# nikhilTkur/Multigrid_dolfinx

Measured on AMD Instinct MI355X. Metric: V-cycles/sec + achieved HBM GB/s, 3D Poisson P1 1024³ DoF, 1/2/4/8 MI355X, higher is better.
Workload: dtype f64

## Files before the change

### multigrid_dolfinx_amd/csrc/mg_capi.hip

```cpp
#include "../../include/mg_hip.h"
#include "mg_kernels.hip.h"
#include "mg_direct.hip.h"
#include "mg_jacobi2.hip.h"
#include "mg_jacobik3d.hip.h"
#include "mg_jacobiblk.hip.h"
#include "mg_lattice.hip.h"

#include <dlfcn.h>
#include <rccl/rccl.h>

#include <algorithm>
#include <array>
#include <cmath>
#include <cstdio>
#include <cstdlib>
#include <cstring>
#include <string>
#include <vector>

using namespace mgk;

namespace {

thread_local std::string g_err;
// ... 174 lines not shown
    int restriction = MG_RESTRICT_INJECTION, smoother = MG_SMOOTH_JACOBI;
    double coarse_rtol = 1e-14;
    int coarse_maxit = 20000;
    int keep_err = 0;
    int use_codes = 1;
    int use_sdia = 1;
    int strip_slices = 64;
    int nontemporal = 1;
    int lds_pad = 32768;
    int rows_per_lane = 2;
    unsigned chunk = 8;
    int pcg_chunk = 16;
    double* partials = nullptr;
    double* scalars = nullptr;
    int* done = nullptr;
    double* h_scalars = nullptr;
    double *pcg_r = nullptr, *pcg_z = nullptr, *pcg_q = nullptr, *pcg_part_a = nullptr, *pcg_part_b = nullptr;
    DVector pcg_p;
    int pcg_parts = 0, pcg_parts_a = 0;
    int pcg_predict = 0;
    int use_graph = 1;
    int comm_priority = 1;
    int lattice_march = 1;
    int64_t lattice_march_min_rows = 1 << 22;
    int lattice_gs2 = 0;
    int lattice_tile = 0;
    int lattice_segments = 0;
    int slab_pair_form = 0;
    int graph_comm = 0;
    uint64_t epoch = 1;
    std::vector<CycleGraph> graphs;
    int use_direct = 1;
    int require_diagonal = 1;
    int fuse_restrict = 1;
    int fuse_block = 1;
    int64_t fuse_block_min_rows = (int64_t)1 << 15, fuse_block_max_rows = (int64_t)1 << 23;
    int fuse_block_k = 0, fuse_block_ez = 11;
    int direct_block_rows = 2048;
    int fuse_2d_lines = 0;
    int gen_odd_rows = 0;
    int cls_escape = 1;
    int storage_auto = 1;
    int storage_qbits = 0;
    int use_classes = 1;
    int fuse_sweeps = 1;
    int64_t fuse_min_rows = (int64_t)1 << 24;
    int fuse_segments = 0;
    int fuse_nontemporal = 0;
    int fuse_classes = 1;
    int fuse_plain_shape = 0;
    int fuse_plain = 2;
    int class_sweeps = 1;
    int fuse_k = 5;
    int fuse_k_shape = 7;
    int fuse_k_segments = 0;
    int timing_force_form = -1;
    int64_t fuse_k_slab_min_rows = (int64_t)1 << 20;
    int fuse_k_slab_min_sweeps = 4;
    int64_t fuse_k_min_rows = (int64_t)1 << 24;
    int64_t fuse_k_small_rows = (int64_t)1 << 22;
    int64_t fuse_k5_min_rows = (int64_t)1 << 26;
    int64_t fuse_k4_min_rows = 0;
    int fuse_k_nt_store = 0;
    int fuse_k_tail = 1;
    int fuse_k_small_tiles = 0;
    int fuse_k_pf = 1;
    int fuse_k_dpp = 1;
    std::vector<const void*> large_lds_kernels;
    int fuse_shape = 1;
    int fuse_wi = 0;
    int fuse_even = 0;
    int march_sweeps = 1;
    int64_t march_min_rows = (int64_t)1 << 22;
    int march_shape = 0;
    int64_t fuse_small_2d_rows = 2048;
    int fuse_small = 1;
    int fuse_2d = 1;
    int fuse_2d_k = 5;
    int fuse_xcd_chunk = 32;
    int cls_blocks_per_cu = 4;
    DirectSolver direct;
    int* ptab_count = nullptr;
    int* rtab_count = nullptr;
    int* rtab_off = nullptr;
    double* rtab_w = nullptr;
    int rtab_m = 0;
    int* ptab_off = nullptr;
    double* ptab_w = nullptr;
    Level mass;
    int mass_level = -1;
    DVector mass_out, diff, uexact;
    int uexact_level = -1;
    int64_t uploads = 0, downloads = 0, graph_replays = 0;
    struct SmootherCount { int64_t launches = 0, sweeps = 0, tail = 0; };
    std::vector<std::array<SmootherCount, MG_PATH_COUNT>> smoother_counts;
    int jk3_tail = 0;
    double* stage = nullptr;
    int64_t stage_elems = 0;
    int64_t bytes = 0;
    Comm comm;
    hipDeviceProp_t prop{};
};

namespace {

constexpr int kMaxParts = 1024;

// ... 876 lines not shown
    L.cls_halo = 1;
    return 0;
}

bool sweepsk_ok(const mg_context* c, const Level& L, bool ignore_size = false) {
    if (c->fuse_k < 3 || !L.cls || !c->fuse_classes) return false;
    if (L.cls_escape) {
        if (L.esc_kmax < 3) return false;
        ignore_size = true;
    }
    const bool slab = !L.replicated && c->comm.active();
    if (slab && (L.hd < 2 || L.cls_halo < 0 || c->halo_planes != 1)) return false;
    if (!ignore_size && (slab ? min_slab_rows(L) < c->fuse_k_slab_min_rows : L.nloc < c->fuse_k_min_rows)) return false;
    return fused_sweeps_ok(c, L, true) && L.g.nk >= 8;
}

int sweepsk_max(const mg_context* c, const Level& L) {
    const int k = std::min(std::min(c->fuse_k, 5), L.nloc < c->fuse_k4_min_rows ? 3 : L.nloc < c->fuse_k_small_rows ? 5 : L.nloc < c->fuse_k5_min_rows ? 4 : 5);
    return L.cls_escape ? std::min(k, L.esc_kmax) : k;
}

template <int K>
int escape_window_k(mg_context* c, const Level& L, const unsigned char* cls, int64_t clead, unsigned* most) {
    constexpr int WI = 64 - 2 * K, HY = 16 * 2 - 2 * K + 2;
    JK3WindowArgs a{};
    a.cls = cls; a.clead = clead; a.P = L.g.plane; a.nx = L.g.nx; a.ny = L.g.ny; a.nz = L.g.nk;
    a.ntx = (a.nx + WI - 1) / WI; a.nty = (a.ny + HY - 1) / HY;
    a.most = reinterpret_cast<unsigned*>(c->partials);
    HIP_TRY(hipMemsetAsync(a.most, 0, sizeof(unsigned), c->stream));
    hipLaunchKernelGGL((jk3_escape_window<K, 16, 2, 1>), dim3((unsigned)(a.ntx * a.nty)), dim3(256), 0, c->stream, a);
    HIP_TRY(hipGetLastError());
    HIP_TRY(hipMemcpyAsync(most, a.most, sizeof(unsigned), hipMemcpyDeviceToHost, c->stream));
    HIP_TRY(hipStreamSynchronize(c->stream));
    if (std::getenv("MG_DEBUG_STORAGE"))
        std::fprintf(stderr, "[mg] escape rows: at most %u in %d planes of a tile (%d sweeps per pass, pool of %d)\n", *most, K + 2, K, jk3_pool(K));
    return 0;
}

int escape_kmax(mg_context* c, const Level& L, const unsigned char* cls, int64_t clead, int* kmax) {
    *kmax = 0;
    if (L.wu != 4 || L.g.nk < 8 || L.g.nx < 32 || L.g.ny < 32) return 0;
    unsigned most = 0;
    MG_TRY(escape_window_k<5>(c, L, cls, clead, &most));
    if (most <= (unsigned)jk3_pool(5)) { *kmax = 5; return 0; }
    MG_TRY(escape_window_k<4>(c, L, cls, clead, &most));
    if (most <= (unsigned)jk3_pool(4)) { *kmax = 4; return 0; }
    MG_TRY(escape_window_k<3>(c, L, cls, clead, &most));
    if (most <= (unsigned)jk3_pool(3)) *kmax = 3;
    return 0;
}

struct JK3Range { int za0, za1, zb0, zb1; };

template <int K, int NW, int LPW, int M, bool DPP, int PF = 1, int WPE = (NW == 12 ? 3 : 2), int TR = 256, bool ESC = false>
int launch_jacobikc_t(mg_context* c, JK3Args a, bool finest, const JK3Range& zr, int seglen) {
    constexpr int EX = 64 * M, EY = NW * LPW, WI = EX - 2 * K, HY = EY - 2 * K + 2;
    a.ntx = (a.nx + WI - 1) / WI;
    a.nty = (a.ny + HY - 1) / HY;
    const int64_t ntile = (int64_t)a.ntx * a.nty;
    constexpr size_t lds = jk3_lds_bytes<K, NW, LPW, M, TR, ESC>();
    static_assert(lds <= 160 * 1024, "one CU's LDS");
    a.za0 = zr.za0; a.za1 = zr.za1; a.zb0 = zr.zb0; a.zb1 = zr.zb1;
    const int planes = std::max(0, zr.za1 - zr.za0) + std::max(0, zr.zb1 - zr.zb0);
    if (planes <= 0) return 0;
    a.ta = (int)ntile; a.seglen_b = 1;
    int64_t items = 0;
    if (seglen <= 0) {
        int64_t cus = std::max(1, c->prop.multiProcessorCount) * (int64_t)std::max<size_t>(1, std::min<size_t>(160 * 1024 / lds, (size_t)(4 * WPE / NW)));
        if (c->fuse_k_tail > 1) cus = c->fuse_k_tail;
        const double warm = 1.4 * K;
        int best = 1, best_ta = (int)ntile, best_m = 1;
        double best_cost = 1e300;
        const bool tail = c->fuse_k_tail && zr.zb1 <= zr.zb0;
        for (int n = 1; n <= std::max(1, planes / 8); ++n) {
            const int len = (planes + n - 1) / n;
            const int64_t full = ntile * n / cus;
            int64_t ta = tail ? std::min<int64_t>(ntile, full * cus / n) : ntile;
            if (ta <= 0 || (ntile - ta) * 2 > cus) ta = ntile;
            const int64_t tb = ntile - ta;
            const int m = tb > 0 ? (int)std::max<int64_t>(1, std::min<int64_t>(cus / tb, planes / 4)) : 1;
            const double cost = (double)((ta * n + cus - 1) / cus) * (len + warm) + (tb > 0 ? (planes + m - 1) / m + warm : 0.0);
            if (cost < best_cost) { best_cost = cost; best = n; best_ta = (int)ta; best_m = m; }
        }
        if (c->fuse_k_segments > 0) { best = std::min(c->fuse_k_segments, planes); best_ta = (int)ntile; }
        seglen = (planes + best - 1) / best;
        a.ta = best_ta;
        a.seglen_b = best_ta < ntile ? (planes + best_m - 1) / best_m : 1;
    }
    a.seglen = seglen;
    {
        const int nseg = (std::max(0, zr.za1 - zr.za0) + seglen - 1) / seglen + (std::max(0, zr.zb1 - zr.zb0) + seglen - 1) / seglen;
        items = (int64_t)a.ta * nseg;
        if (a.ta < ntile) items += (ntile - a.ta) * (int64_t)((planes + a.seglen_b - 1) / a.seglen_b);
    }
    if (items >= ((int64_t)1 << 31) - 4096) return fail("too many tiles");
    a.nitems = (unsigned)items;
    a.xcd_chunk = (unsigned)c->fuse_xcd_chunk;
    const int64_t group = 8 * (int64_t)a.xcd_chunk;
    const unsigned grid = (unsigned)(((items + group - 1) / group) * group);
    if (a.ncls > TR) return fail("more row classes than this tile shape keeps in LDS");
    void (*kern)(JK3Args) = finest ? sdia_jacobikc_finest<K, NW, LPW, M, DPP, PF, WPE, TR> : sdia_jacobikc<K, NW, LPW, M, DPP, PF, WPE, TR>;
    if constexpr (ESC) kern = sdia_jacobikc_escape<K, NW, LPW, M, DPP, PF, WPE, TR>;
    MG_TRY(allow_large_lds(c, reinterpret_cast<const void*>(kern), lds));
    hipLaunchKernelGGL(kern, dim3(grid), dim3(NW * WAVE), lds, c->stream, a);
    HIP_TRY(hipGetLastError());
    c->jk3_tail = a.ta < ntile ? 1 : 0;
    return 0;
}

template <int K, int PF>
int launch_jacobikc_kp(mg_context* c, const JK3Args& a, bool finest, const JK3Range& zr, int seglen) {
    if (!c->fuse_k_dpp) return launch_jacobikc_t<K, 12, 2, 2, false, PF>(c, a, finest, zr, seglen);
    int shape = c->fuse_k_shape >= 3 && a.ncls > 64 ? 1 : c->fuse_k_shape;
    if (shape == 1 && a.ncls <= 64 && K <= 4 && c->fuse_k_small_tiles) {
        constexpr int WI = 64 - 2 * K, HY = 48 - 2 * K + 2;
        if ((int64_t)((a.nx + WI - 1) / WI) * ((a.ny + HY - 1) / HY) < std::max(1, c->prop.multiProcessorCount)) shape = 4;
    }
    switch (shape) {
        case 1: return launch_jacobikc_t<K, 12, 4, 1, true, PF>(c, a, finest, zr, seglen);
        case 2: return launch_jacobikc_t<K, 8, 3, 2, true, PF>(c, a, finest, zr, seglen);
        case 3: return launch_jacobikc_t<K, 6, 4, 1, true, PF, 3, 64>(c, a, finest, zr, seglen);
        case 4: return launch_jacobikc_t<K, 8, 3, 1, true, PF, 4, 64>(c, a, finest, zr, seglen);
        case 5: if constexpr (K <= 4) return launch_jacobikc_t<K, 4, 6, 1, true, PF, 2, 64>(c, a, finest, zr, seglen);
        case 6: if constexpr (K <= 4 && PF == 1) return launch_jacobikc_t<K, 16, 3, 1, true, 1, 4>(c, a, finest, zr, seglen);
        case 7: return launch_jacobikc_t<K, 16, 2, 1, true, PF, 4>(c, a, finest, zr, seglen);
        default: return launch_jacobikc_t<K, 12, 2, 2, true, PF>(c, a, finest, zr, seglen);
    }
}

template <int K>
int launch_jacobikc_k(mg_context* c, const JK3Args& a, bool finest, const JK3Range& zr, int seglen) {
    if (a.escape) {
        if constexpr (K >= 3) return launch_jacobikc_t<K, 16, 2, 1, true, 1, 4, 256, true>(c, a, finest, zr, seglen);
        else return fail("levels with escape rows take three to five sweeps per pass");
    }
    if constexpr (K == 3 || K == 4) {
        if (c->fuse_k_pf == 2 && (K == 3 || c->fuse_k_shape == 7)) return launch_jacobikc_kp<K, 2>(c, a, finest, zr, seglen);
    }
    if constexpr (K == 2) return launch_jacobikc_t<K, 12, 4, 1, true, 1>(c, a, finest, zr, seglen);
    else return launch_jacobikc_kp<K, 1>(c, a, finest, zr, seglen);
}

int launch_jacobikc(mg_context* c, const Level& L, int K, const double* x_rows, const double* f_rows, double* out_rows,
                    const JK3Range* zr = nullptr, int seglen = 0) {
    JK3Args a{};
    a.x = x_rows; a.f = f_rows; a.out = out_rows;
    a.cls = L.cls; a.ctab = L.ctab; a.clead = L.cls_lead; a.ncls = L.ncls; a.cmain = L.cmain;
    for (int t = 0; t < 8; ++t) a.cm[t] = L.cm[t];
    a.P = L.g.plane; a.nx = L.g.nx; a.ny = L.g.ny; a.nz = L.g.nk; a.omega = c->omega;
    const bool dist = !L.replicated && c->comm.active();
    a.plo = dist && c->comm.rank > 0 ? K : 0;
    a.phi = dist && c->comm.rank + 1 < c->comm.world ? K : 0;
    if (dist && (L.hd < K || L.cls_halo != 1)) return fail("the level's halos are not prepared for that many sweeps per pass");
    if (L.cls_escape && K > L.esc_kmax) return fail("too many escape rows per tile for that many sweeps per pass");
    a.force_form = c->timing_force_form;
    a.nt_store = c->fuse_k_nt_store;
    a.escape = L.cls_escape ? 1 : 0; a.dvals = L.dvals; a.mlead = L.mlead; a.sshift = L.R == 1 ? 6 : (L.R == 2 ? 7 : 8);
    const JK3Range whole{0, L.g.nk, 0, 0};
    const bool finest = c->nlev > 1 && &L == &c->L[c->nlev - 1];
    c->jk3_tail = 0;
    switch (K) {
        case 2: return launch_jacobikc_k<2>(c, a, finest, zr ? *zr : whole, seglen);
        case 3: return launch_jacobikc_k<3>(c, a, finest, zr ? *zr : whole, seglen);
        case 4: return launch_jacobikc_k<4>(c, a, finest, zr ? *zr : whole, seglen);
        case 5: return launch_jacobikc_k<5>(c, a, finest, zr ? *zr : whole, seglen);
        default: return fail("sweeps per pass must be in 2..5");
    }
}

int check_coloring(mg_context* c, Level& L) {
    EllArgs a{};
    a.vals = L.vals; a.cols = L.cols; a.codes = L.codes; a.offsets = L.offsets; a.W = L.W;
    a.nloc = L.nloc; a.lead = L.g.lead; a.dinv = L.dinv; a.color_kind = COLOR_LATTICE9; a.grow0 = L.row0; a.gnx = L.g.nx; a.gny = L.g.ny;
    int* d_flag = reinterpret_cast<int*>(c->partials);
    HIP_TRY(hipMemsetAsync(d_flag, 0, sizeof(int), c->stream));
    const dim3 grid(blocks_for(L.nloc, 256)), blk(256);
    if (L.sdia) {
        a.vals = L.dvals; a.mlead = L.mlead;
        for (int t = 0; t < 8; ++t) a.up[t] = L.up[t];
        switch (L.R) {
            case 1: hipLaunchKernelGGL(sdia_check_coloring<1>, grid, blk, 0, c->stream, a, L.wu, d_flag); break;
            case 2: hipLaunchKernelGGL(sdia_check_coloring<2>, grid, blk, 0, c->stream, a, L.wu, d_flag); break;
            default: hipLaunchKernelGGL(sdia_check_coloring<4>, grid, blk, 0, c->stream, a, L.wu, d_flag); break;
        }
    } else {
        switch (L.R) {
            case 1: hipLaunchKernelGGL(ell_check_coloring<1>, grid, blk, 0, c->stream, a, L.nslices, d_flag); break;
            case 2: hipLaunchKernelGGL(ell_check_coloring<2>, grid, blk, 0, c->stream, a, L.nslices, d_flag); break;
            default: hipLaunchKernelGGL(ell_check_coloring<4>, grid, blk, 0, c->stream, a, L.nslices, d_flag); break;
        }
// ... 1600 lines not shown
    } else if (k == "fuse_shape") {
        if (value < 0 || value > 3) return fail("fuse_shape must be 0..3");
        c->fuse_shape = (int)value;
    } else if (k == "march_sweeps") {
        c->march_sweeps = value != 0;
    } else if (k == "march_min_rows") {
        c->march_min_rows = value;
    } else if (k == "march_shape") {
        if (value < 0 || value > 1) return fail("march_shape must be 0 or 1");
        c->march_shape = (int)value;
    } else if (k == "fuse_small_2d_rows") {
        c->fuse_small_2d_rows = value;
    } else if (k == "fuse_small") {
        c->fuse_small = value != 0;
    } else if (k == "fuse_2d") {
        c->fuse_2d = value != 0;
    } else if (k == "fuse_2d_k") {
        if (value < 2 || value > 5) return fail("fuse_2d_k must be in 2..5");
        c->fuse_2d_k = (int)value;
    } else if (k == "lattice_march") {
        c->lattice_march = value != 0;
    } else if (k == "lattice_march_min_rows") {
        c->lattice_march_min_rows = value;
    } else if (k == "lattice_gs2") {
        c->lattice_gs2 = value != 0;
    } else if (k == "lattice_tile") {
        if (value < 0 || value > 2) return fail("lattice_tile must be 0, 1 or 2");
        c->lattice_tile = (int)value;
    } else if (k == "lattice_segments") {
        if (value < 0 || value > 4096) return fail("lattice_segments must be in 0..4096");
        c->lattice_segments = (int)value;
    } else if (k == "fuse_xcd_chunk") {
        if (value < 1 || value > 512) return fail("fuse_xcd_chunk must be in 1..512");
        c->fuse_xcd_chunk = (int)value;
    } else if (k == "cls_blocks_per_cu") {
        if (value < 1 || value > 64) return fail("cls_blocks_per_cu must be in 1..64");
        c->cls_blocks_per_cu = (int)value;
    } else if (k == "fuse_wi") {
        c->fuse_wi = (int)value;
    } else if (k == "fuse_even") {
        c->fuse_even = value != 0;
    } else if (k == "class_sweeps") {
        c->class_sweeps = value != 0;
    } else if (k == "fuse_plain_shape") {
        if (value < 0 || value > 2) return fail("fuse_plain_shape must be 0..2");
        c->fuse_plain_shape = (int)value;
    } else if (k == "fuse_plain") {
        if (value != 1 && value != 2) return fail("fuse_plain must be 1 or 2");
        c->fuse_plain = (int)value;
    } else if (k == "fuse_k") {
        if (value < 0 || value > 5) return fail("fuse_k must be in 0..5 (below 3: pairs of sweeps only)");
        c->fuse_k = (int)value;
    } else if (k == "fuse_k_shape") {
        if (value < 0 || value > 7) return fail("fuse_k_shape must be 0..7");
        c->fuse_k_shape = (int)value;
    } else if (k == "fuse_k_slab_min_rows") {
        c->fuse_k_slab_min_rows = value;
    } else if (k == "fuse_k_slab_min_sweeps") {
        if (value < 2) return fail("fuse_k_slab_min_sweeps must be at least 2");
        c->fuse_k_slab_min_sweeps = (int)value;
    } else if (k == "fuse_k_min_rows") {
        c->fuse_k_min_rows = value;
    } else if (k == "fuse_k_small_rows") {
        c->fuse_k_small_rows = value;
    } else if (k == "fuse_k5_min_rows") {
        c->fuse_k5_min_rows = value;
    } else if (k == "fuse_k4_min_rows") {
        c->fuse_k4_min_rows = value;
    } else if (k == "fuse_k_nt_store") {
        c->fuse_k_nt_store = value != 0;
    } else if (k == "fuse_k_tail") {
        if (value < 0) return fail("fuse_k_tail must be >= 0");
        c->fuse_k_tail = (int)value;
    } else if (k == "fuse_k_small_tiles") {
        c->fuse_k_small_tiles = value != 0;
    } else if (k == "fuse_k_pf") {
        if (value != 1 && value != 2) return fail("fuse_k_pf must be 1 or 2");
        c->fuse_k_pf = (int)value;
    } else if (k == "fuse_k_dpp") {
        c->fuse_k_dpp = value != 0;
    } else if (k == "fuse_k_segments") {
        if (value < 0) return fail("fuse_k_segments must be >= 0");
        c->fuse_k_segments = (int)value;
    } else if (k == "fuse_classes") {
        c->fuse_classes = value != 0;
    } else if (k == "fuse_nontemporal") {
        c->fuse_nontemporal = value != 0;
    } else if (k == "fuse_segments") {
        if (value < 0) return fail("fuse_segments must be >= 0");
        c->fuse_segments = (int)value;
    } else if (k == "coarse_direct") {
        c->use_direct = value != 0;
        free_direct(c);
    } else if (k == "pcg_chunk") {
        if (value < 1) return fail("pcg_chunk must be positive");
        c->pcg_chunk = (int)value;
    } else {
        return fail("unknown tuning key " + k);
    }
    return 0;
}

namespace {

struct DevTemp {
    void* p = nullptr;
    DevTemp() = default;
// ... 823 lines not shown
```

### multigrid_dolfinx_amd/csrc/mg_jacobik3d.hip.h

```cpp
#pragma once
#include "mg_jacobi2.hip.h"
#include <type_traits>

namespace mgk {

struct JK3Args {
    const double* x;
    const double* f;
    double* out;
    const unsigned char* cls;
    const double* ctab;
    int64_t clead, P;
    int ncls, cmain;
    double cm[8];
    double omega;
    int nx, ny, nz;
    int plo, phi;
    int ntx, nty, seglen, za0, za1, zb0, zb1;
    int ta, seglen_b;
    unsigned nitems, xcd_chunk;
    int nt_store;
    int escape;
    const double* dvals;
    int64_t mlead;
    int sshift;
    int force_form;
};

constexpr int jk3_pool(int K) { return K >= 5 ? 512 : 1024; }

template <int K, int NW, int LPW, int M, int TR> constexpr size_t jk3_lds_doubles() {
    return TR * CLS_W + (size_t)K * (NW * LPW + 2) * (64 * M) + 2 * (64 * M + 2);
}
template <int K, int NW, int LPW, int M, int TR, bool ESC = false> constexpr size_t jk3_lds_bytes() {
    constexpr size_t base = jk3_lds_doubles<K, NW, LPW, M, TR>();
    return sizeof(double) * (ESC ? (base + CLS_W - 1) / CLS_W * CLS_W + (size_t)(jk3_pool(K) + 1) * CLS_W : base);
}


template <int K, int NW, int LPW, int M, bool DPP, int PF, int TR, bool ESC = false>
__device__ __forceinline__ void jk3_body(const JK3Args& a) {
    constexpr int EX = 64 * M, EY = NW * LPW, NC = M * LPW, IMG = (EY + 2) * EX;
    constexpr int CBITS = ESC ? 16 : 8, CPR = 32 / CBITS, CW = (NC + CPR - 1) / CPR;
    constexpr unsigned CMASK = (1u << CBITS) - 1u;
    constexpr int DYN0 = (int)((jk3_lds_doubles<K, NW, LPW, M, TR>() + CLS_W - 1) / CLS_W);
    static_assert(CLS_W == 8, "table rows of eight doubles");
    constexpr int WI = EX - 2 * K, HY = EY - 2 * K + 2;
    static_assert(NC * (K + 1) <= 64, "the fast-path flags live in one scalar register pair");
    static_assert(WI > 0 && HY > 0, "tile too small for K sweeps");
    static_assert(PF == 1 || PF == 2, "planes of x in flight");
    extern __shared__ double j2_smem[];
    double* const sT = j2_smem;
    double* const sI = sT + TR * CLS_W + (EX + 2);
    const int lane = threadIdx.x & 63;
    const int wave = __builtin_amdgcn_readfirstlane((int)(threadIdx.x >> 6));

    unsigned id;
    {
        const unsigned b = blockIdx.x, xcd = b & 7u, j = b >> 3, ch = a.xcd_chunk;
        id = ((j / ch) * 8u + xcd) * ch + (j % ch);
    }
    if (id >= a.nitems) return;
    const unsigned ntile = (unsigned)(a.ntx * a.nty);
    const int nsa = (a.za1 - a.za0 + a.seglen - 1) / a.seglen;
    const int nsb = (a.zb1 - a.zb0 + a.seglen - 1) / a.seglen;
    const unsigned items_a = (unsigned)a.ta * (unsigned)(nsa + max(nsb, 0));
    unsigned tt;
    int z0, z1;
    if (id < items_a) {
        const int seg = (int)(id / (unsigned)a.ta);
        tt = id % (unsigned)a.ta;
        z0 = seg < nsa ? a.za0 + seg * a.seglen : a.zb0 + (seg - nsa) * a.seglen;
        z1 = min(seg < nsa ? a.za1 : a.zb1, z0 + a.seglen);
    } else {
        const unsigned j = id - items_a, tb = ntile - (unsigned)a.ta;
        tt = (unsigned)a.ta + j % tb;
        z0 = a.za0 + (int)(j / tb) * a.seglen_b;
        z1 = min(a.za1, z0 + a.seglen_b);
    }
    const int tiy = (int)(tt / (unsigned)a.ntx), tix = (int)(tt % (unsigned)a.ntx);
    if (z1 <= z0) return;
    const int tx0 = tix * WI - K, ty0 = tiy * HY - (K - 1);

    {
        const int nt = a.ncls * CLS_W;
        for (int i = threadIdx.x; i < nt; i += NW * WAVE) {
            double v = a.ctab[i];
            if ((i & (CLS_W - 1)) == CLS_W - 1) {
                const double d = a.ctab[i - 4];
                v = a.omega * (1.0 / (d != 0.0 ? d : 1.0));
            }
            sT[i] = v;
        }
        for (int i = threadIdx.x; i < K * IMG + 2 * (EX + 2); i += NW * WAVE) sT[TR * CLS_W + i] = 0.0;
    }
    unsigned* const esc_count = reinterpret_cast<unsigned*>(sT + (size_t)CLS_W * (DYN0 + jk3_pool(K)));
    if constexpr (ESC) {
        if (threadIdx.x == 0) *esc_count = 0u;
    }
    const double m0 = a.cm[0], m1 = a.cm[1], m2 = a.cm[2], m3 = a.cm[3], m4 = a.cm[4], m5 = a.cm[5], m6 = a.cm[6];
    const double mcf = a.omega * (1.0 / (m3 != 0.0 ? m3 : 1.0));
    const int cmain = a.cmain;

    const int ey0 = wave * LPW;
    const int lw0 = (ey0 + 1) * EX + lane;
    auto lwof = [&](int c) -> int { return (c / M) * EX + 64 * (c % M); };
    int ibase[(K + 1) / 2];
#pragma unroll
    for (int q = 0; q < (K + 1) / 2; ++q) {
        ibase[q] = 2 * q * IMG + lw0;
        asm volatile("" : "+v"(ibase[q]));
    }
    auto image = [&](int t) -> double* { return sI + ibase[t >> 1] + (t & 1) * IMG; };
    unsigned inT = 0;
    const int64_t rb0 = (int64_t)(ty0 + ey0) * a.nx + (tx0 + lane);
    auto rowof = [&](int c) -> int64_t { return rb0 + (int64_t)(c / M) * a.nx + 64 * (c % M); };
    unsigned shw = 0;
#pragma unroll
    for (int c = 0; c < NC; ++c) {
        const int ex = lane + 64 * (c % M), ey = ey0 + c / M;
        if (ex >= K && ex < EX - K && ey >= K - 1 && ey <= EY - K && tx0 + ex < a.nx && ty0 + ey < a.ny) inT |= 1u << c;
        const int64_t r = rowof(c);
        shw |= (r < 0 ? 0u : (r >= a.P ? 2u : 1u)) << (2 * c);
    }
    auto shof = [&](int c) -> int { return (int)((shw >> (2 * c)) & 3u) - 1; };
    unsigned standin = 0;
#pragma unroll
    for (int c = 0; c < NC; ++c) {
        const int line = ty0 + ey0 + c / M;
        if (lane + 64 * (c % M) > a.nx + 1 - tx0 || line < -2 || line > a.ny + 1) standin |= 1u << c;
    }
    const bool wlo = wave == 0, whi = wave == NW - 1;

    const int bias = 2 * a.nx + K + 2;
    const int xcl = a.nx + 1 - tx0;
    unsigned eo[NC], eor[M];
#pragma unroll
    for (int c = 0; c < NC; ++c)
        eo[c] = 8u * (unsigned)(min(max(ty0 + ey0 + c / M, -2), a.ny + 1) * a.nx + tx0 + min(lane + 64 * (c % M), xcl) + bias);
#pragma unroll
    for (int r = 0; r < M; ++r)
        eor[r] = 8u * (unsigned)((wlo ? max(ty0 - 1, -2) : min(ty0 + EY, a.ny + 1)) * a.nx + tx0 + min(lane + 64 * r, xcl) + bias);
    const unsigned char* const clsb = a.cls + a.clead - bias;
    const double* const xb0 = a.x - bias;
    const double* const fb0 = a.f - bias;
    auto sbase = [](const void* p) -> gcptr_t {
        const unsigned long long u = (unsigned long long)p;
        const unsigned lo = (unsigned)__builtin_amdgcn_readfirstlane((int)(unsigned)u);
        const unsigned hi = (unsigned)__builtin_amdgcn_readfirstlane((int)(unsigned)(u >> 32));
        return (gcptr_t)(((unsigned long long)hi << 32) | lo);
    };
    auto ldd = [](gcptr_t b, unsigned e8) -> double {
        asm volatile("" : "+v"(e8));
        return *(const __attribute__((address_space(1))) double*)(b + e8);
    };
    typedef unsigned int __attribute__((aligned(1))) u32_unaligned_t;
    auto ldc = [](gcptr_t b, unsigned e8) -> int {
        unsigned e = e8 >> 3;
        asm volatile("" : "+v"(e));
        return (int)*(const __attribute__((address_space(1))) u32_unaligned_t*)(b + e);
    };
    const int pmin = -a.plo - 1, pmax = a.nz + a.phi;

    double acc[K][NC], fr[K][NC];
    double XA[NC], XB[PF == 2 ? NC : 1], hyA[M], hyB[PF == 2 ? M : 1];
    int CA[NC], CB[PF == 2 ? NC : 1];
    double FN[PF == 2 ? NC : 1];
    unsigned cw[K + 1][CW];
    unsigned long long fast = 0;
    constexpr unsigned long long ALLFAST = (NC * (K + 1) == 64) ? ~0ull : ((1ull << (NC * (K + 1))) - 1ull);
#pragma unroll
    for (int c = 0; c < NC; ++c) {
#pragma unroll
        for (int t = 0; t < K; ++t) acc[t][c] = fr[t][c] = 0.0;
        XA[c] = 0.0;
        CA[c] = 0;
    }
#pragma unroll
    for (int j = 0; j <= K; ++j)
#pragma unroll
        for (int q = 0; q < CW; ++q) cw[j][q] = 0u;
#pragma unroll
    for (int r = 0; r < M; ++r) hyA[r] = 0.0;
    XB[0] = 0.0; hyB[0] = 0.0; CB[0] = 0; FN[0] = 0.0;

    auto load_slice = [&](const int i, const int n, const int plane, const int fplane, double (&X)[NC], int (&C)[NC], double (&hy)[M])
        __attribute__((always_inline)) {
        const int64_t o = (int64_t)min(max(plane, pmin), pmax) * a.P;
        const gcptr_t cb = sbase(clsb + o);
        const gcptr_t xb = sbase(xb0 + o);
        const gcptr_t fb = sbase(fb0 + (int64_t)min(max(fplane, pmin), pmax) * a.P);
#pragma unroll
        for (int c = 0; c < NC; ++c) {
            if ((c * n) / NC != i) continue;
            X[c] = ldd(xb, eo[c]);
            C[c] = ldc(cb, eo[c]);
            if constexpr (PF == 2) FN[c] = ldd(fb, eo[c]);
            else fr[K - 1][c] = ldd(fb, eo[c]);
        }
        if (i == n - 1 && (wlo || whi)) {
#pragma unroll
            for (int r = 0; r < M; ++r) hy[r] = ldd(xb, eor[r]);
        }
    };
    auto cls_of = [&](int j, int c) -> int { return (int)((cw[j][c / CPR] >> (CBITS * (c % CPR))) & CMASK); };
    auto cls_now = [&](int j, int c) -> int {
        unsigned w = cw[j][c / CPR];
        asm volatile("" : "+v"(w));
        return (int)((w >> (CBITS * (c % CPR))) & CMASK);
    };
    int k_plane = 0;
    bool k_store = false;
    __attribute__((address_space(1))) char* k_out = nullptr;
    auto store = [&](int c, double v) {
        unsigned e8 = eo[c];
        asm volatile("" : "+v"(e8));
        if (a.nt_store) __builtin_nontemporal_store(v, (__attribute__((address_space(1))) double*)(k_out + e8));
        else *(__attribute__((address_space(1))) double*)(k_out + e8) = v;
    };
    int lo_t[K + 1], n_t[K + 1];
#pragma unroll
    for (int t = 1; t <= K; ++t) {
        lo_t[t] = -min(a.plo, K - t);
        n_t[t] = a.nz + min(a.phi, K - t) - lo_t[t];
    }

    auto phase_a_fast = [&](auto col_tag, const double (&X)[NC]) __attribute__((always_inline)) {
        constexpr bool COL = decltype(col_tag)::value;
#pragma unroll
        for (int r = 0; r < M; ++r) {
#pragma unroll
            for (int l = 0; l < LPW; ++l) {
                const int c = l * M + r, iw = lwof(c);
                double k0 = m0, k6 = m6, kcf = mcf;
                if constexpr (COL) {
                    const dvec2_t* const tr = reinterpret_cast<const dvec2_t*>(sT + CLS_W * cls_of(0, c));
                    const dvec2_t t01 = tr[0], t67 = tr[3];
                    k0 = t01.x; k6 = t67.x; kcf = t67.y;
                }
                double nw = X[c];
#pragma unroll
                for (int t = 1; t <= K; ++t) {
                    double* const img = image(t - 1);
                    const double wd = img[iw];
                    const double s = fma(k6, nw, acc[t - 1][c]);
                    const double o = wd + kcf * (fr[K - t][c] - s);
                    acc[t - 1][c] = fma(k0, wd, 0.0);
                    img[iw] = nw;
                    nw = o;
                }
                if (k_store && (inT >> c & 1u)) store(c, nw);
            }
        }
    };
    auto phase_b_fast = [&](auto col_tag, const int t) __attribute__((always_inline)) {
        constexpr bool COL = decltype(col_tag)::value;
        const double* const img = image(t - 1);
        double v[LPW][M], ys[M], yn[M];
#pragma unroll
        for (int r = 0; r < M; ++r) {
            ys[r] = img[-EX + 64 * r];
#pragma unroll
            for (int l = 0; l < LPW; ++l) v[l][r] = img[l * EX + 64 * r];
            yn[r] = img[LPW * EX + 64 * r];
        }
#pragma unroll
        for (int l = 0; l < LPW; ++l) {
            double yw[M], ye[M];
            if constexpr (DPP) {
                double fw[M], fe[M];
#pragma unroll
                for (int r = 0; r < M; ++r) { fw[r] = jk3_from_west(v[l][r]); fe[r] = jk3_from_east(v[l][r]); }
#pragma unroll
                for (int r = 0; r < M; ++r) {
                    yw[r] = (r > 0 && lane == 0) ? fw[r > 0 ? r - 1 : 0] : fw[r];
                    ye[r] = (r + 1 < M && lane == 63) ? fe[r + 1 < M ? r + 1 : r] : fe[r];
                }
            } else {
#pragma unroll
                for (int r = 0; r < M; ++r) {
                    yw[r] = img[l * EX + 64 * r - 1];
                    ye[r] = img[l * EX + 64 * r + 1];
                }
            }
#pragma unroll
            for (int r = 0; r < M; ++r) {
                const int c = l * M + r;
                double k1 = m1, k2 = m2, k3 = m3, k4 = m4, k5 = m5;
                if constexpr (COL) {
                    const dvec2_t* const tr = reinterpret_cast<const dvec2_t*>(sT + CLS_W * cls_of(0, c));
                    const dvec2_t t01 = tr[0], t23 = tr[1], t45 = tr[2];
                    k1 = t01.y; k2 = t23.x; k3 = t23.y; k4 = t45.x; k5 = t45.y;
                }
                double s = acc[t - 1][c];
                s = fma(k1, l > 0 ? v[l > 0 ? l - 1 : 0][r] : ys[r], s);
                s = fma(k2, yw[r], s);
                s = fma(k3, v[l][r], s);
                s = fma(k4, ye[r], s);
                s = fma(k5, l + 1 < LPW ? v[l + 1 < LPW ? l + 1 : l][r] : yn[r], s);
                acc[t - 1][c] = s;
            }
        }
    };
    auto phase_a_general = [&](const double (&X)[NC]) __attribute__((always_inline)) {
#pragma unroll
        for (int c = 0; c < NC; ++c) {
            const int iw = lwof(c);
            double nw = X[c];
            int pc = k_plane + shof(c);
            asm volatile("" : "+v"(pc));
#pragma unroll
            for (int t = 1; t <= K; ++t) {
                const int j = K - t;
                double* const img = image(t - 1);
                const double wd = img[iw];
                const dvec2_t t67 = reinterpret_cast<const dvec2_t*>(sT + CLS_W * cls_now(j, c))[3];
                const dvec2_t t01 = reinterpret_cast<const dvec2_t*>(sT + CLS_W * cls_now(j + 1, c))[0];
                const double s = fma(t67.x, nw, acc[t - 1][c]);
                double o = wd + t67.y * (fr[j][c] - s);
                o = (unsigned)(pc + j - lo_t[t]) < (unsigned)n_t[t] ? o : 0.0;
                acc[t - 1][c] = fma(t01.x, wd, 0.0);
                img[iw] = nw;
                nw = o;
                __builtin_amdgcn_sched_barrier(0);
            }
            if (k_store && (inT >> c & 1u)) store(c, nw);
        }
    };
    auto phase_b_general = [&](const int t) __attribute__((always_inline)) {
#pragma unroll
        for (int c = 0; c < NC; ++c) {
            const int iw = lwof(c);
            const double* const img = image(t - 1);
            const double ys = img[iw - EX], yw = img[iw - 1], yd = img[iw], ye = img[iw + 1], yn = img[iw + EX];
            const dvec2_t* const tr = reinterpret_cast<const dvec2_t*>(sT + CLS_W * cls_now(K - t, c));
            const dvec2_t t01 = tr[0], t23 = tr[1], t45 = tr[2];
            double s = acc[t - 1][c];
            s = fma(t01.y, ys, s);
            s = fma(t23.x, yw, s);
            s = fma(t23.y, yd, s);
            s = fma(t45.x, ye, s);
            s = fma(t45.y, yn, s);
            acc[t - 1][c] = s;
            __builtin_amdgcn_sched_barrier(0);
        }
    };

    auto step = [&](const int k, double (&X)[NC], int (&C)[NC], double (&hy)[M], double (&XN)[PF == 2 ? NC : 1],
                    int (&CN)[PF == 2 ? NC : 1], double (&hyN)[PF == 2 ? M : 1]) __attribute__((always_inline)) {
        k_plane = k; k_store = k >= z0;
        {
            const unsigned long long u = (unsigned long long)(a.out - bias + (int64_t)k * a.P);
            const unsigned lo = (unsigned)__builtin_amdgcn_readfirstlane((int)(unsigned)u);
            const unsigned hi = (unsigned)__builtin_amdgcn_readfirstlane((int)(unsigned)(u >> 32));
            k_out = (__attribute__((address_space(1))) char*)(((unsigned long long)hi << 32) | lo);
        }
#pragma unroll
        for (int c = 0; c < NC; ++c) {
            asm volatile("" : "+v"(C[c]));
            asm volatile("" : "+v"(X[c]));
            C[c] &= 255;
        }
        if constexpr (ESC) {
            if (a.escape) {
                const int64_t mp = (int64_t)min(max(k + K, pmin), pmax) * a.P - bias + a.mlead;
                const int sh = a.sshift;
                const double* const dv = a.dvals;
                auto at = [&](int64_t m, int slot) -> double { return dv[((((m >> sh) << 2) + slot) << sh) + (m & (((int64_t)1 << sh) - 1))]; };
                unsigned long long em[NC];
                unsigned total = 0u;
#pragma unroll
                for (int c = 0; c < NC; ++c) {
                    if (C[c] == CLS_ESCAPE && (standin >> c & 1u)) C[c] = 0;
                    em[c] = __ballot(C[c] == CLS_ESCAPE);
                    total += (unsigned)__popcll(em[c]);
                }
                if (total != 0u) {
                    unsigned b0 = 0u;
                    if (lane == 0) b0 = atomicAdd(esc_count, total);
                    b0 = (unsigned)__builtin_amdgcn_readfirstlane((int)b0);
                    double e[NC][7];
#pragma unroll
                    for (int c = 0; c < NC; ++c) {
                        if (C[c] == CLS_ESCAPE) {
                            const int64_t m = mp + (int64_t)(eo[c] >> 3);
                            e[c][0] = at(m - a.P, 3); e[c][1] = at(m - a.nx, 2); e[c][2] = at(m - 1, 1);
                            e[c][3] = at(m, 0); e[c][4] = at(m, 1); e[c][5] = at(m, 2); e[c][6] = at(m, 3);
                        }
                    }
#pragma unroll
                    for (int c = 0; c < NC; ++c) {
                        if (C[c] == CLS_ESCAPE) {
                            const unsigned below = __builtin_amdgcn_mbcnt_hi((unsigned)(em[c] >> 32), __builtin_amdgcn_mbcnt_lo((unsigned)em[c], 0u));
                            const int row = DYN0 + (int)((b0 + below) & (unsigned)(jk3_pool(K) - 1));
                            double* const tr = sT + CLS_W * row;
#pragma unroll
                            for (int i = 0; i < 7; ++i) tr[i] = e[c][i];
                            tr[7] = a.omega * (1.0 / (e[c][3] != 0.0 ? e[c][3] : 1.0));
                            C[c] = row;
                        }
                        b0 += (unsigned)__popcll(em[c]);
                    }
                }
            }
        }
        {
            unsigned m = 0;
#pragma unroll
            for (int q = 0; q < CW; ++q) cw[K][q] = 0u;
#pragma unroll
            for (int c = 0; c < NC; ++c) {
                cw[K][c / CPR] |= (unsigned)C[c] << (CBITS * (c % CPR));
                if (__builtin_amdgcn_readfirstlane((int)(__ballot(C[c] != cmain) == 0ull))) m |= 1u << c;
            }
            fast |= (unsigned long long)m << (K * NC);
        }
        int form = 2;
        if ((a.plo > 0 || k >= 1) && (a.phi > 0 || k + K + 1 < a.nz)) {
            if (fast == ALLFAST) {
                form = 0;
            } else {
                bool same = true;
#pragma unroll
                for (int j = 0; j <= K; ++j)
#pragma unroll
                    for (int c = 0; c < NC; ++c) same = same && cls_of(j, c) == cls_of(0, c);
                if (__builtin_amdgcn_readfirstlane((int)(__ballot(!same) == 0ull))) form = 1;
            }
        }
        if (a.force_form >= 0) form = a.force_form;
        if (form == 0) phase_a_fast(std::false_type{}, X);
        else if (form == 1) phase_a_fast(std::true_type{}, X);
        else phase_a_general(X);
        if (wlo || whi) {
            double* const ring = image(0) + (wlo ? -EX : LPW * EX);
#pragma unroll
            for (int r = 0; r < M; ++r) ring[64 * r] = hy[r];
        }
#pragma unroll
        for (int c = 0; c < NC; ++c) {
#pragma unroll
            for (int j = 0; j + 1 < K; ++j) fr[j][c] = fr[j + 1][c];
            asm volatile("" : "+v"(fr[K - 2][c]));
        }
#pragma unroll
        for (int j = 0; j < K; ++j)
#pragma unroll
            for (int q = 0; q < CW; ++q) cw[j][q] = cw[j + 1][q];
        fast >>= NC;
        __syncthreads();
        if constexpr (PF == 2) {
#pragma unroll
            for (int c = 0; c < NC; ++c) {
                X[c] = XN[c]; C[c] = CN[c]; fr[K - 1][c] = FN[c];
                asm volatile("" : "+v"(X[c]));
                asm volatile("" : "+v"(C[c]));
                asm volatile("" : "+v"(fr[K - 1][c]));
            }
            if (wlo || whi) {
#pragma unroll
                for (int r = 0; r < M; ++r) { hy[r] = hyN[r]; asm volatile("" : "+v"(hy[r])); }
            }
        }
        auto issue = [&](const int i, const int n) __attribute__((always_inline)) {
            __builtin_amdgcn_sched_barrier(0);
            if constexpr (PF == 2) load_slice(i, n, k + K + 2, k + K + 1, XN, CN, hyN);
            else load_slice(i, n, k + K + 1, k + K, X, C, hy);
            __builtin_amdgcn_sched_barrier(0);
        };
#pragma unroll
        for (int t = 1; t <= K; ++t) {
            if (form == 0) phase_b_fast(std::false_type{}, t);
            else if (form == 1) phase_b_fast(std::true_type{}, t);
            else phase_b_general(t);
            issue(t - 1, K);
        }
        __syncthreads();
    };

    load_slice(0, 1, z0 - K, z0 - K - 1, XA, CA, hyA);
    if constexpr (PF == 2) {
#pragma unroll
        for (int c = 0; c < NC; ++c) fr[K - 1][c] = FN[c];
        load_slice(0, 1, z0 - K + 1, z0 - K, XB, CB, hyB);
    }
    __syncthreads();

    for (int k = z0 - 2 * K; k < z1; ++k) step(k, XA, CA, hyA, XB, CB, hyB);
}

template <int K, int NW, int LPW, int M, bool DPP, int PF, int WPE, int TR>
__global__ __attribute__((amdgpu_flat_work_group_size(NW * WAVE, NW * WAVE), amdgpu_waves_per_eu(WPE, WPE)))
void sdia_jacobikc(JK3Args a) {
    jk3_body<K, NW, LPW, M, DPP, PF, TR>(a);
}

template <int K, int NW, int LPW, int M, bool DPP, int PF, int WPE, int TR>
__global__ __attribute__((amdgpu_flat_work_group_size(NW * WAVE, NW * WAVE), amdgpu_waves_per_eu(WPE, WPE)))
void sdia_jacobikc_finest(JK3Args a) {
    jk3_body<K, NW, LPW, M, DPP, PF, TR>(a);
}

template <int K, int NW, int LPW, int M, bool DPP, int PF, int WPE, int TR>
__global__ __attribute__((amdgpu_flat_work_group_size(NW * WAVE, NW * WAVE), amdgpu_waves_per_eu(WPE, WPE)))
void sdia_jacobikc_escape(JK3Args a) {
    jk3_body<K, NW, LPW, M, DPP, PF, TR, true>(a);
}

struct JK3WindowArgs {
    const unsigned char* cls;
    int64_t clead, P;
    int nx, ny, nz, ntx, nty;
    unsigned* most;
};

template <int K, int NW, int LPW, int M>
__global__ __launch_bounds__(256) void jk3_escape_window(JK3WindowArgs a) {
    constexpr int EX = 64 * M, EY = NW * LPW, WI = EX - 2 * K, HY = EY - 2 * K + 2, W = K + 2;
    __shared__ unsigned s_ring[W], s_plane;
    const int tiy = (int)(blockIdx.x / (unsigned)a.ntx), tix = (int)(blockIdx.x % (unsigned)a.ntx);
    const int tx0 = tix * WI - K, ty0 = tiy * HY - (K - 1), xcl = a.nx + 1 - tx0;
    unsigned win = 0u, best = 0u;
    for (int p = 0; p < a.nz; ++p) {
        if (threadIdx.x == 0) s_plane = 0u;
        __syncthreads();
        unsigned n = 0u;
        for (int i = threadIdx.x; i < EX * EY; i += 256) {
            const int ex = i % EX, line = ty0 + i / EX;
            if (ex > xcl || line < -2 || line > a.ny + 1) continue;
            const int64_t row = (int64_t)p * a.P + (int64_t)line * a.nx + tx0 + ex;
            n += a.cls[a.clead + row] == CLS_ESCAPE ? 1u : 0u;
        }
        if (n) atomicAdd(&s_plane, n);
        __syncthreads();
        if (threadIdx.x == 0) {
            win += s_plane - (p >= W ? s_ring[p % W] : 0u);
            s_ring[p % W] = s_plane;
            best = max(best, win);
        }
    }
    if (threadIdx.x == 0 && best) atomicMax(a.most, best);
}

}
```

Before: 4.157.

## Add one-barrier-per-step fused Jacobi kernel variant with double-buffered LDS images

Adds a B1 variant of the K-sweep fused 3D Jacobi kernel. It keeps the first sweep's plane of x in registers, with south and north halo rows loaded directly from global memory. The remaining sweep images are double-buffered in LDS, alternating by plane parity, so the trailing __syncthreads per plane step can be dropped. The new default shape selector uses this variant (shape 8) when a pass fuses five sweeps, and keeps shape 7 otherwise. In exchange it needs more LDS for the double buffering and more registers, which may reduce occupancy.

```diff
diff --git a/multigrid_dolfinx_amd/csrc/mg_capi.hip b/multigrid_dolfinx_amd/csrc/mg_capi.hip
--- a/multigrid_dolfinx_amd/csrc/mg_capi.hip
+++ b/multigrid_dolfinx_amd/csrc/mg_capi.hip
@@ -250,7 +250,7 @@
     int fuse_plain = 2;
     int class_sweeps = 1;
     int fuse_k = 5;
-    int fuse_k_shape = 7;
+    int fuse_k_shape = -1;
     int fuse_k_segments = 0;
     int timing_force_form = -1;
     int64_t fuse_k_slab_min_rows = (int64_t)1 << 20;
@@ -1233,13 +1233,17 @@
 
 struct JK3Range { int za0, za1, zb0, zb1; };
 
-template <int K, int NW, int LPW, int M, bool DPP, int PF = 1, int WPE = (NW == 12 ? 3 : 2), int TR = 256, bool ESC = false>
+int jk3_shape(const mg_context* c, int K) {
+    return c->fuse_k_shape >= 0 ? c->fuse_k_shape : (K >= 5 ? 8 : 7);
+}
+
+template <int K, int NW, int LPW, int M, bool DPP, int PF = 1, int WPE = (NW == 12 ? 3 : 2), int TR = 256, bool ESC = false, bool B1 = false>
 int launch_jacobikc_t(mg_context* c, JK3Args a, bool finest, const JK3Range& zr, int seglen) {
     constexpr int EX = 64 * M, EY = NW * LPW, WI = EX - 2 * K, HY = EY - 2 * K + 2;
     a.ntx = (a.nx + WI - 1) / WI;
     a.nty = (a.ny + HY - 1) / HY;
     const int64_t ntile = (int64_t)a.ntx * a.nty;
-    constexpr size_t lds = jk3_lds_bytes<K, NW, LPW, M, TR, ESC>();
+    constexpr size_t lds = B1 ? jk3b_lds_bytes<K, NW, LPW, M, TR>() : jk3_lds_bytes<K, NW, LPW, M, TR, ESC>();
     static_assert(lds <= 160 * 1024, "one CU's LDS");
     a.za0 = zr.za0; a.za1 = zr.za1; a.zb0 = zr.zb0; a.zb1 = zr.zb1;
     const int planes = std::max(0, zr.za1 - zr.za0) + std::max(0, zr.zb1 - zr.zb0);
@@ -1280,8 +1284,10 @@
     const int64_t group = 8 * (int64_t)a.xcd_chunk;
     const unsigned grid = (unsigned)(((items + group - 1) / group) * group);
     if (a.ncls > TR) return fail("more row classes than this tile shape keeps in LDS");
-    void (*kern)(JK3Args) = finest ? sdia_jacobikc_finest<K, NW, LPW, M, DPP, PF, WPE, TR> : sdia_jacobikc<K, NW, LPW, M, DPP, PF, WPE, TR>;
+    void (*kern)(JK3Args) = nullptr;
     if constexpr (ESC) kern = sdia_jacobikc_escape<K, NW, LPW, M, DPP, PF, WPE, TR>;
+    else if constexpr (B1) kern = finest ? sdia_jacobikc_finest_b1<K, NW, LPW, M, WPE, TR> : sdia_jacobikc_b1<K, NW, LPW, M, WPE, TR>;
+    else kern = finest ? sdia_jacobikc_finest<K, NW, LPW, M, DPP, PF, WPE, TR> : sdia_jacobikc<K, NW, LPW, M, DPP, PF, WPE, TR>;
     MG_TRY(allow_large_lds(c, reinterpret_cast<const void*>(kern), lds));
     hipLaunchKernelGGL(kern, dim3(grid), dim3(NW * WAVE), lds, c->stream, a);
     HIP_TRY(hipGetLastError());
@@ -1292,7 +1298,7 @@
 template <int K, int PF>
 int launch_jacobikc_kp(mg_context* c, const JK3Args& a, bool finest, const JK3Range& zr, int seglen) {
     if (!c->fuse_k_dpp) return launch_jacobikc_t<K, 12, 2, 2, false, PF>(c, a, finest, zr, seglen);
-    int shape = c->fuse_k_shape >= 3 && a.ncls > 64 ? 1 : c->fuse_k_shape;
+    int shape = jk3_shape(c, K) >= 3 && a.ncls > 64 ? 1 : jk3_shape(c, K);
     if (shape == 1 && a.ncls <= 64 && K <= 4 && c->fuse_k_small_tiles) {
         constexpr int WI = 64 - 2 * K, HY = 48 - 2 * K + 2;
         if ((int64_t)((a.nx + WI - 1) / WI) * ((a.ny + HY - 1) / HY) < std::max(1, c->prop.multiProcessorCount)) shape = 4;
@@ -1305,6 +1311,8 @@
         case 5: if constexpr (K <= 4) return launch_jacobikc_t<K, 4, 6, 1, true, PF, 2, 64>(c, a, finest, zr, seglen);
         case 6: if constexpr (K <= 4 && PF == 1) return launch_jacobikc_t<K, 16, 3, 1, true, 1, 4>(c, a, finest, zr, seglen);
         case 7: return launch_jacobikc_t<K, 16, 2, 1, true, PF, 4>(c, a, finest, zr, seglen);
+        case 8: if constexpr (PF == 1) return launch_jacobikc_t<K, 16, 2, 1, true, 1, 4, 256, false, true>(c, a, finest, zr, seglen);
+                else return fail("tile shape 8 stages one plane of x (fuse_k_pf 1)");
         default: return launch_jacobikc_t<K, 12, 2, 2, true, PF>(c, a, finest, zr, seglen);
     }
 }
@@ -1316,7 +1324,7 @@
         else return fail("levels with escape rows take three to five sweeps per pass");
     }
     if constexpr (K == 3 || K == 4) {
-        if (c->fuse_k_pf == 2 && (K == 3 || c->fuse_k_shape == 7)) return launch_jacobikc_kp<K, 2>(c, a, finest, zr, seglen);
+        if (c->fuse_k_pf == 2 && (K == 3 || jk3_shape(c, K) == 7)) return launch_jacobikc_kp<K, 2>(c, a, finest, zr, seglen);
     }
     if constexpr (K == 2) return launch_jacobikc_t<K, 12, 4, 1, true, 1>(c, a, finest, zr, seglen);
     else return launch_jacobikc_kp<K, 1>(c, a, finest, zr, seglen);
@@ -3023,7 +3031,7 @@
         if (value < 0 || value > 5) return fail("fuse_k must be in 0..5 (below 3: pairs of sweeps only)");
         c->fuse_k = (int)value;
     } else if (k == "fuse_k_shape") {
-        if (value < 0 || value > 7) return fail("fuse_k_shape must be 0..7");
+        if (value < -1 || value > 8) return fail("fuse_k_shape must be 0..8, or -1 (by sweeps per pass)");
         c->fuse_k_shape = (int)value;
     } else if (k == "fuse_k_slab_min_rows") {
         c->fuse_k_slab_min_rows = value;
diff --git a/multigrid_dolfinx_amd/csrc/mg_jacobik3d.hip.h b/multigrid_dolfinx_amd/csrc/mg_jacobik3d.hip.h
--- a/multigrid_dolfinx_amd/csrc/mg_jacobik3d.hip.h
+++ b/multigrid_dolfinx_amd/csrc/mg_jacobik3d.hip.h
@@ -32,15 +32,24 @@
 template <int K, int NW, int LPW, int M, int TR> constexpr size_t jk3_lds_doubles() {
     return TR * CLS_W + (size_t)K * (NW * LPW + 2) * (64 * M) + 2 * (64 * M + 2);
 }
+template <int K, int NW, int LPW, int M, int TR> constexpr size_t jk3b_lds_doubles() {
+    return TR * CLS_W + (size_t)(2 * (K - 1) * (NW * LPW + 1) + 1) * (64 * M);
+}
+template <int K, int NW, int LPW, int M, int TR> constexpr size_t jk3b_lds_bytes() {
+    return sizeof(double) * jk3b_lds_doubles<K, NW, LPW, M, TR>();
+}
+
 template <int K, int NW, int LPW, int M, int TR, bool ESC = false> constexpr size_t jk3_lds_bytes() {
     constexpr size_t base = jk3_lds_doubles<K, NW, LPW, M, TR>();
     return sizeof(double) * (ESC ? (base + CLS_W - 1) / CLS_W * CLS_W + (size_t)(jk3_pool(K) + 1) * CLS_W : base);
 }
 
 
-template <int K, int NW, int LPW, int M, bool DPP, int PF, int TR, bool ESC = false>
+template <int K, int NW, int LPW, int M, bool DPP, int PF, int TR, bool ESC = false, bool B1 = false>
 __device__ __forceinline__ void jk3_body(const JK3Args& a) {
     constexpr int EX = 64 * M, EY = NW * LPW, NC = M * LPW, IMG = (EY + 2) * EX;
+    constexpr int IS = (EY + 1) * EX, PS = (K - 1) * IS;
+    static_assert(!B1 || (DPP && PF == 1 && !ESC), "one barrier per step: DPP neighbours, one plane of x in flight, no escape rows");
     constexpr int CBITS = ESC ? 16 : 8, CPR = 32 / CBITS, CW = (NC + CPR - 1) / CPR;
     constexpr unsigned CMASK = (1u << CBITS) - 1u;
     constexpr int DYN0 = (int)((jk3_lds_doubles<K, NW, LPW, M, TR>() + CLS_W - 1) / CLS_W);
@@ -92,7 +101,8 @@
             }
             sT[i] = v;
         }
-        for (int i = threadIdx.x; i < K * IMG + 2 * (EX + 2); i += NW * WAVE) sT[TR * CLS_W + i] = 0.0;
+        constexpr int NZ = B1 ? (2 * (K - 1) * (EY + 1) + 1) * EX : K * IMG + 2 * (EX + 2);
+        for (int i = threadIdx.x; i < NZ; i += NW * WAVE) sT[TR * CLS_W + i] = 0.0;
     }
     unsigned* const esc_count = reinterpret_cast<unsigned*>(sT + (size_t)CLS_W * (DYN0 + jk3_pool(K)));
     if constexpr (ESC) {
@@ -112,6 +122,10 @@
         asm volatile("" : "+v"(ibase[q]));
     }
     auto image = [&](int t) -> double* { return sI + ibase[t >> 1] + (t & 1) * IMG; };
+    int bcur = 0, bprev = 0;
+    auto limg = [&](int base, int t) -> double* { return j2_smem + base + (t - 1) * IS + EX; };
+    double XP[B1 ? NC : 1];
+    double hS[M], hN[M];
     unsigned inT = 0;
     const int64_t rb0 = (int64_t)(ty0 + ey0) * a.nx + (tx0 + lane);
     auto rowof = [&](int c) -> int64_t { return rb0 + (int64_t)(c / M) * a.nx + 64 * (c % M); };
@@ -141,6 +155,14 @@
 #pragma unroll
     for (int r = 0; r < M; ++r)
         eor[r] = 8u * (unsigned)((wlo ? max(ty0 - 1, -2) : min(ty0 + EY, a.ny + 1)) * a.nx + tx0 + min(lane + 64 * r, xcl) + bias);
+    unsigned eos[B1 ? M : 1], eon[B1 ? M : 1];
+    if constexpr (B1) {
+#pragma unroll
+        for (int r = 0; r < M; ++r) {
+            eos[r] = 8u * (unsigned)(min(max(ty0 + ey0 - 1, -2), a.ny + 1) * a.nx + tx0 + min(lane + 64 * r, xcl) + bias);
+            eon[r] = 8u * (unsigned)(min(max(ty0 + ey0 + LPW, -2), a.ny + 1) * a.nx + tx0 + min(lane + 64 * r, xcl) + bias);
+        }
+    }
     const unsigned char* const clsb = a.cls + a.clead - bias;
     const double* const xb0 = a.x - bias;
     const double* const fb0 = a.f - bias;
@@ -181,8 +203,10 @@
 #pragma unroll
         for (int q = 0; q < CW; ++q) cw[j][q] = 0u;
 #pragma unroll
-    for (int r = 0; r < M; ++r) hyA[r] = 0.0;
+    for (int r = 0; r < M; ++r) hyA[r] = hS[r] = hN[r] = 0.0;
     XB[0] = 0.0; hyB[0] = 0.0; CB[0] = 0; FN[0] = 0.0;
+#pragma unroll
+    for (int c = 0; c < (B1 ? NC : 1); ++c) XP[c] = 0.0;
 
     auto load_slice = [&](const int i, const int n, const int plane, const int fplane, double (&X)[NC], int (&C)[NC], double (&hy)[M])
         __attribute__((always_inline)) {
@@ -198,7 +222,12 @@
             if constexpr (PF == 2) FN[c] = ldd(fb, eo[c]);
             else fr[K - 1][c] = ldd(fb, eo[c]);
         }
-        if (i == n - 1 && (wlo || whi)) {
+        if constexpr (B1) {
+            if (i == n - 1) {
+#pragma unroll
+                for (int r = 0; r < M; ++r) { hS[r] = ldd(xb, eos[r]); hN[r] = ldd(xb, eon[r]); }
+            }
+        } else if (i == n - 1 && (wlo || whi)) {
 #pragma unroll
             for (int r = 0; r < M; ++r) hy[r] = ldd(xb, eor[r]);
         }
@@ -241,6 +270,15 @@
                 double nw = X[c];
 #pragma unroll
                 for (int t = 1; t <= K; ++t) {
+                    if constexpr (B1) {
+                        const double wd = t == 1 ? XP[c] : limg(bprev, t - 1)[iw];
+                        const double s = fma(k6, nw, acc[t - 1][c]);
+                        const double o = wd + kcf * (fr[K - t][c] - s);
+                        acc[t - 1][c] = fma(k0, wd, 0.0);
+                        if (t > 1) limg(bcur, t - 1)[iw] = nw;
+                        nw = o;
+                        continue;
+                    }
                     double* const img = image(t - 1);
                     const double wd = img[iw];
                     const double s = fma(k6, nw, acc[t - 1][c]);
@@ -253,12 +291,19 @@
             }
         }
     };
-    auto phase_b_fast = [&](auto col_tag, const int t) __attribute__((always_inline)) {
+    auto phase_b_fast = [&](auto col_tag, const int t, const double (&X)[NC]) __attribute__((always_inline)) {
         constexpr bool COL = decltype(col_tag)::value;
-        const double* const img = image(t - 1);
+        const double* const img = B1 ? limg(bcur, t > 1 ? t - 1 : 1) : image(t - 1);
         double v[LPW][M], ys[M], yn[M];
 #pragma unroll
         for (int r = 0; r < M; ++r) {
+            if (B1 && t == 1) {
+                ys[r] = hS[r];
+#pragma unroll
+                for (int l = 0; l < LPW; ++l) v[l][r] = X[l * M + r];
+                yn[r] = hN[r];
+                continue;
+            }
             ys[r] = img[-EX + 64 * r];
 #pragma unroll
             for (int l = 0; l < LPW; ++l) v[l][r] = img[l * EX + 64 * r];
@@ -312,27 +357,49 @@
 #pragma unroll
             for (int t = 1; t <= K; ++t) {
                 const int j = K - t;
-                double* const img = image(t - 1);
-                const double wd = img[iw];
+                double* const img = B1 ? limg(bcur, t > 1 ? t - 1 : 1) : image(t - 1);
+                const double wd = B1 ? (t == 1 ? XP[B1 ? c : 0] : limg(bprev, t - 1)[iw]) : img[iw];
                 const dvec2_t t67 = reinterpret_cast<const dvec2_t*>(sT + CLS_W * cls_now(j, c))[3];
                 const dvec2_t t01 = reinterpret_cast<const dvec2_t*>(sT + CLS_W * cls_now(j + 1, c))[0];
                 const double s = fma(t67.x, nw, acc[t - 1][c]);
                 double o = wd + t67.y * (fr[j][c] - s);
                 o = (unsigned)(pc + j - lo_t[t]) < (unsigned)n_t[t] ? o : 0.0;
                 acc[t - 1][c] = fma(t01.x, wd, 0.0);
-                img[iw] = nw;
+                if (!B1 || t > 1) img[iw] = nw;
                 nw = o;
                 __builtin_amdgcn_sched_barrier(0);
             }
             if (k_store && (inT >> c & 1u)) store(c, nw);
         }
     };
-    auto phase_b_general = [&](const int t) __attribute__((always_inline)) {
+    auto phase_b_general = [&](const int t, const double (&X)[NC]) __attribute__((always_inline)) {
+        double x0w[B1 ? NC : 1], x0e[B1 ? NC : 1];
+        if constexpr (B1) {
+            if (t == 1) {
+                double fw[NC], fe[NC];
+#pragma unroll
+                for (int c = 0; c < NC; ++c) { fw[c] = jk3_from_west(X[c]); fe[c] = jk3_from_east(X[c]); }
+#pragma unroll
+                for (int c = 0; c < NC; ++c) {
+                    const int r = c % M;
+                    x0w[c] = (r > 0 && lane == 0) ? fw[r > 0 ? c - 1 : c] : fw[c];
+                    x0e[c] = (r + 1 < M && lane == 63) ? fe[r + 1 < M ? c + 1 : c] : fe[c];
+                }
+            }
+        }
 #pragma unroll
         for (int c = 0; c < NC; ++c) {
             const int iw = lwof(c);
-            const double* const img = image(t - 1);
-            const double ys = img[iw - EX], yw = img[iw - 1], yd = img[iw], ye = img[iw + 1], yn = img[iw + EX];
+            double ys, yw, yd, ye, yn;
+            if (B1 && t == 1) {
+                const int l = c / M, r = c % M;
+                ys = l > 0 ? X[l > 0 ? c - M : c] : hS[r];
+                yw = x0w[B1 ? c : 0]; yd = X[c]; ye = x0e[B1 ? c : 0];
+                yn = l + 1 < LPW ? X[l + 1 < LPW ? c + M : c] : hN[r];
+            } else {
+                const double* const img = B1 ? limg(bcur, t > 1 ? t - 1 : 1) : image(t - 1);
+                ys = img[iw - EX]; yw = img[iw - 1]; yd = img[iw]; ye = img[iw + 1]; yn = img[iw + EX];
+            }
             const dvec2_t* const tr = reinterpret_cast<const dvec2_t*>(sT + CLS_W * cls_now(K - t, c));
             const dvec2_t t01 = tr[0], t23 = tr[1], t45 = tr[2];
             double s = acc[t - 1][c];
@@ -349,6 +416,12 @@
     auto step = [&](const int k, double (&X)[NC], int (&C)[NC], double (&hy)[M], double (&XN)[PF == 2 ? NC : 1],
                     int (&CN)[PF == 2 ? NC : 1], double (&hyN)[PF == 2 ? M : 1]) __attribute__((always_inline)) {
         k_plane = k; k_store = k >= z0;
+        if constexpr (B1) {
+            bcur = TR * CLS_W + ey0 * EX + lane + (k & 1) * PS;
+            bprev = TR * CLS_W + ey0 * EX + lane + ((k + 1) & 1) * PS;
+            asm volatile("" : "+v"(bcur));
+            asm volatile("" : "+v"(bprev));
+        }
         {
             const unsigned long long u = (unsigned long long)(a.out - bias + (int64_t)k * a.P);
             const unsigned lo = (unsigned)__builtin_amdgcn_readfirstlane((int)(unsigned)u);
@@ -432,7 +505,10 @@
         if (form == 0) phase_a_fast(std::false_type{}, X);
         else if (form == 1) phase_a_fast(std::true_type{}, X);
         else phase_a_general(X);
-        if (wlo || whi) {
+        if constexpr (B1) {
+#pragma unroll
+            for (int c = 0; c < NC; ++c) XP[c] = X[c];
+        } else if (wlo || whi) {
             double* const ring = image(0) + (wlo ? -EX : LPW * EX);
 #pragma unroll
             for (int r = 0; r < M; ++r) ring[64 * r] = hy[r];
@@ -470,12 +546,12 @@
         };
 #pragma unroll
         for (int t = 1; t <= K; ++t) {
-            if (form == 0) phase_b_fast(std::false_type{}, t);
-            else if (form == 1) phase_b_fast(std::true_type{}, t);
-            else phase_b_general(t);
+            if (form == 0) phase_b_fast(std::false_type{}, t, X);
+            else if (form == 1) phase_b_fast(std::true_type{}, t, X);
+            else phase_b_general(t, X);
             issue(t - 1, K);
         }
-        __syncthreads();
+        if constexpr (!B1) __syncthreads();
     };
 
     load_slice(0, 1, z0 - K, z0 - K - 1, XA, CA, hyA);
@@ -499,6 +575,17 @@
 __global__ __attribute__((amdgpu_flat_work_group_size(NW * WAVE, NW * WAVE), amdgpu_waves_per_eu(WPE, WPE)))
 void sdia_jacobikc_finest(JK3Args a) {
     jk3_body<K, NW, LPW, M, DPP, PF, TR>(a);
+}
+
+template <int K, int NW, int LPW, int M, int WPE, int TR>
+__global__ __attribute__((amdgpu_flat_work_group_size(NW * WAVE, NW * WAVE), amdgpu_waves_per_eu(WPE, WPE)))
+void sdia_jacobikc_b1(JK3Args a) {
+    jk3_body<K, NW, LPW, M, true, 1, TR, false, true>(a);
+}
+template <int K, int NW, int LPW, int M, int WPE, int TR>
+__global__ __attribute__((amdgpu_flat_work_group_size(NW * WAVE, NW * WAVE), amdgpu_waves_per_eu(WPE, WPE)))
+void sdia_jacobikc_finest_b1(JK3Args a) {
+    jk3_body<K, NW, LPW, M, true, 1, TR, false, true>(a);
 }
 
 template <int K, int NW, int LPW, int M, bool DPP, int PF, int WPE, int TR>
```

Result: faster. 4.366 (median of 6 runs) (+5.0%).
